# dfdazac/blp

Measured on AMD Instinct MI355X. Metric: scored triples/sec, all-entity eval (raw + filtered ranks, MRR + Hits@k), higher is better.
Workload: dtype f32; 1 GPU; fb15k237-transe; rel_model=transe, entities=14541, dim=128, triples_per_ranking_call=52870, filter_graph_edges=310116, parallelism=single GPU, ranks_in_process_group=1

## Files before the change

blp_amd/csrc/exact_coop.h:

```cpp
#pragma once
#include <hip/hip_runtime.h>
#include <stdint.h>

#include "rank_common.h"
#include "score_core.h"
#include "table_elem.h"

#pragma clang fp contract(off)

namespace blp {

constexpr int kRefStride = 36;

template <class TE>
struct RowOf {
    const TE* p;
    __device__ __forceinline__ float operator[](int k) const { return (float)p[k]; }
};

template <class T>
__device__ __forceinline__ const T* shfl_ptr(const T* p, int src) {
    const unsigned long long v = reinterpret_cast<unsigned long long>(p);
    const unsigned lo = __shfl((unsigned)v, src), hi = __shfl((unsigned)(v >> 32), src);
    return reinterpret_cast<const T*>(((unsigned long long)hi << 32) | lo);
}

template <class T>
__device__ __forceinline__ void gather_chunk(float (&x)[32], const T* const (&g)[8], int s, float* slab, int lane) {
#pragma unroll
    for (int i = 0; i < 8; ++i) {
        const float4 v = load4<T>(g[i] + 32 * s);
        x[4 * i] = v.x; x[4 * i + 1] = v.y; x[4 * i + 2] = v.z; x[4 * i + 3] = v.w;
    }
    float* wr = slab + (lane >> 3) * kRefStride + (lane & 7) * 4;
    wave_lds_sync();
#pragma unroll
    for (int i = 0; i < 8; ++i)
        *reinterpret_cast<float4*>(wr + 8 * i * kRefStride) = make_float4(x[4 * i], x[4 * i + 1], x[4 * i + 2], x[4 * i + 3]);
    wave_lds_sync();
    const float* rd = slab + lane * kRefStride;
#pragma unroll
    for (int j = 0; j < 8; ++j) {
        const float4 w = *reinterpret_cast<const float4*>(rd + 4 * j);
        x[4 * j] = w.x; x[4 * j + 1] = w.y; x[4 * j + 2] = w.z; x[4 * j + 3] = w.w;
    }
}


template <int D, class TE = float>
__device__ __forceinline__ float transe_key_64(const TE* pe, const float* pf, const float* pr, bool head, float* slab, int lane) {
    const int sub_row = lane >> 3, sub_col = (lane & 7) * 4;
    const TE* ge[8];
    const float* gf[8];
    const float* gr[8];
#pragma unroll
    for (int k = 0; k < 8; ++k) {
        ge[k] = shfl_ptr(pe, 8 * k + sub_row) + sub_col;
        gf[k] = shfl_ptr(pf, 8 * k + sub_row) + sub_col;
        gr[k] = shfl_ptr(pr, 8 * k + sub_row) + sub_col;
    }
    float sum = 0.0f;
#pragma unroll
    for (int s = 0; s < D / 32; ++s) {
        float e[32], f[32], r[32];
        gather_chunk(e, ge, s, slab, lane);
        gather_chunk(f, gf, s, slab, lane);
        gather_chunk(r, gr, s, slab, lane);
#pragma unroll
        for (int k = 0; k < 32; ++k) {
            float x = (head ? e[k] : f[k]) + r[k];
            x = x - (head ? f[k] : e[k]);
            sum = sum + fabsf(x);
        }
    }
    return -sum;
}

template <class TE = float>
__device__ __forceinline__ void gather_issue_rt(float (&x)[32], const TE* const (&g)[8], int s, int cols, int lane) {
    const bool mine = (lane & 7) * 4 < cols;
#pragma unroll
    for (int i = 0; i < 8; ++i) {
        float4 v = make_float4(0.f, 0.f, 0.f, 0.f);
        if (mine) v = load4<TE>(g[i] + 32 * s);
        x[4 * i] = v.x; x[4 * i + 1] = v.y; x[4 * i + 2] = v.z; x[4 * i + 3] = v.w;
    }
}
__device__ __forceinline__ void gather_transpose(float (&x)[32], float* slab, int lane) {
    float* wr = slab + (lane >> 3) * kRefStride + (lane & 7) * 4;
    wave_lds_sync();
#pragma unroll
    for (int i = 0; i < 8; ++i)
        *reinterpret_cast<float4*>(wr + 8 * i * kRefStride) = make_float4(x[4 * i], x[4 * i + 1], x[4 * i + 2], x[4 * i + 3]);
    wave_lds_sync();
    const float* rd = slab + lane * kRefStride;
#pragma unroll
    for (int j = 0; j < 8; ++j) {
        const float4 w = *reinterpret_cast<const float4*>(rd + 4 * j);
        x[4 * j] = w.x; x[4 * j + 1] = w.y; x[4 * j + 2] = w.z; x[4 * j + 3] = w.w;
    }
}

__device__ __forceinline__ float transe_key_64_rt(const float* pe, const float* pf, const float* pr, int D, bool head,
                                                  float* slab, int lane) {
    const int sub_row = lane >> 3, sub_col = (lane & 7) * 4;
    const float* ge[8];
    const float* gf[8];
    const float* gr[8];
#pragma unroll
    for (int k = 0; k < 8; ++k) {
        ge[k] = shfl_ptr(pe, 8 * k + sub_row) + sub_col;
        gf[k] = shfl_ptr(pf, 8 * k + sub_row) + sub_col;
        gr[k] = shfl_ptr(pr, 8 * k + sub_row) + sub_col;
    }
    float sum = 0.0f;
    for (int s = 0; s * 32 < D; ++s) {
        const int cols = D - 32 * s < 32 ? D - 32 * s : 32;
        float e[32], f[32], r[32];
        gather_issue_rt(e, ge, s, cols, lane);
        gather_issue_rt(f, gf, s, cols, lane);
        gather_issue_rt(r, gr, s, cols, lane);
        gather_transpose(e, slab, lane);
        gather_transpose(f, slab, lane);
        gather_transpose(r, slab, lane);
#pragma unroll
        for (int k = 0; k < 32; ++k) {
            float x = (head ? e[k] : f[k]) + r[k];
            x = x - (head ? f[k] : e[k]);
            if (k < cols) sum = sum + fabsf(x);
        }
    }
    return -sum;
}

__device__ __forceinline__ void stage_query_rt(const float* __restrict__ f, const float* __restrict__ r, int D, bool head,
                                               float* qa, float* qb, int lane) {
    for (int c = 4 * lane; c < D; c += 256) {
        const float4 fv = *reinterpret_cast<const float4*>(f + c);
        const float4 rv = *reinterpret_cast<const float4*>(r + c);
        if (head) {
            *reinterpret_cast<float4*>(qa + c) = rv;
            *reinterpret_cast<float4*>(qb + c) = fv;
        } else {
            *reinterpret_cast<float4*>(qa + c) = make_float4(fv.x + rv.x, fv.y + rv.y, fv.z + rv.z, fv.w + rv.w);
        }
    }
}

template <class TE = float>
__device__ __forceinline__ float transe_key_64_one_query_rt(const TE* pe, const float* qa, const float* qb, int D, bool head,
                                                            float* slab, int lane) {
    const int sub_row = lane >> 3, sub_col = (lane & 7) * 4;
    const TE* ge[8];
#pragma unroll
    for (int k = 0; k < 8; ++k) ge[k] = shfl_ptr(pe, 8 * k + sub_row) + sub_col;
    float sum = 0.0f;
    const int n_chunks = (D + 31) / 32;
    float ring[4][32];
    auto issue = [&](float (&x)[32], int s) {
        const int rest = D - 32 * s;
        gather_issue_rt(x, ge, s, rest < 32 ? rest : 32, lane);
    };
    auto consume = [&](float (&x)[32], int s) {
        gather_transpose(x, slab, lane);
        const float* a = qa + 32 * s;
        const float* b = qb + 32 * s;
        const int cols = D - 32 * s;
#pragma unroll
        for (int k4 = 0; k4 < 8; ++k4) {
            if (4 * k4 < cols) {
                const float4 av = *reinterpret_cast<const float4*>(a + 4 * k4);
                const float as[4] = {av.x, av.y, av.z, av.w};
                if (head) {
                    const float4 bv = *reinterpret_cast<const float4*>(b + 4 * k4);
                    const float bs[4] = {bv.x, bv.y, bv.z, bv.w};
#pragma unroll
                    for (int i = 0; i < 4; ++i) {
                        float v = x[4 * k4 + i] + as[i];
                        v = v - bs[i];
                        sum = sum + fabsf(v);
                    }
                } else {
#pragma unroll
                    for (int i = 0; i < 4; ++i) sum = sum + fabsf(as[i] - x[4 * k4 + i]);
                }
            }
        }
    };
    if (0 < n_chunks) issue(ring[0], 0);
    if (1 < n_chunks) issue(ring[1], 1);
    if (2 < n_chunks) issue(ring[2], 2);
    for (int s0 = 0; s0 < n_chunks; s0 += 4) {
        static_for<4>([&](auto ii) {
            constexpr int i = decltype(ii)::value;
            const int s = s0 + i;
            if (s < n_chunks) {
                if (s + 3 < n_chunks) issue(ring[(i + 3) % 4], s + 3);
                consume(ring[i], s);
            }
        });
    }
    return -sum;
}

template <int MODEL, int SIDE, int D, class TE>
__device__ __forceinline__ float score_term(const TE* __restrict__ ep, const float* __restrict__ f,
                                            const float* __restrict__ r, int i) {
    constexpr int H = D / 2;
    (void)H;
    const RowOf<TE> e{ep};
    if constexpr (MODEL == DISTMULT) {
        if constexpr (SIDE == TAIL) {
            const float c = f[i] * r[i];
            return c * e[i];
        } else {
            const float x = e[i] * r[i];
            return x * f[i];
        }
    } else if constexpr (MODEL == COMPLEX) {
        if constexpr (SIDE == TAIL) {
            const float c0 = r[i] * f[i], c1 = r[i] * f[H + i], c2 = r[H + i] * f[i], c3 = r[H + i] * f[H + i];
            const float a = c0 * e[i];
            const float b = c1 * e[H + i];
            const float cc = c2 * e[H + i];
            const float d = c3 * e[i];
            float s = a + b;
            s = s + cc;
            return s - d;
        } else {
            float a = r[i] * e[i];          a = a * f[i];
            float b = r[i] * e[H + i];      b = b * f[H + i];
            float cc = r[H + i] * e[i];     cc = cc * f[H + i];
            float d = r[H + i] * e[H + i];  d = d * f[i];
            float s = a + b;
            s = s + cc;
            return s - d;
        }
    } else {
        if constexpr (SIDE == TAIL) {
            const float c0 = f[i] * r[i];
            const float a = c0 * e[H + i];
            float b = e[i] * r[H + i];
            b = b * f[H + i];
            return a + b;
        } else {
            float a = e[i] * r[i];
            a = a * f[H + i];
            const float c2 = f[i] * r[H + i];
            const float b = c2 * e[H + i];
            return a + b;
        }
    }
}

template <int MODEL, int SIDE, int D, class TE = float>
__device__ __forceinline__ float coop_score(const TE* __restrict__ e, const float* __restrict__ f,
                                            const float* __restrict__ r, int sub) {
    constexpr int NT = MODEL == DISTMULT ? D : D / 2;
    float a = score_term<MODEL, SIDE, D>(e, f, r, sub);
#pragma unroll
    for (int k = 1; k < NT / 32; ++k) a = a + score_term<MODEL, SIDE, D>(e, f, r, 32 * k + sub);
    float v = a + __shfl_down(a, 8, 32);
    v = v + __shfl_down(a, 16, 32);
    v = v + __shfl_down(a, 24, 32);
    float s = __shfl(v, 0, 32);
#pragma unroll
    for (int l = 1; l < 8; ++l) s = s + __shfl(v, l, 32);
    return MODEL == SIMPLE ? s / 2.0f : s;
}


template <int MODEL, int D>
__device__ __forceinline__ void true_key_lane(const QRows& q_true, const QRows& q_fixed, const QRows& q_rel,
                                              int64_t q, int64_t q_head, float* __restrict__ key_true,
                                              unsigned long long* __restrict__ acc) {
    acc[q] = 0;
    float e[D];
    load_row<D>(e, q_true.row(q));
    const float* f = q_fixed.row(q);
    const float* r = q_rel.row(q);
    key_true[q] = q < q_head ? Scorer<MODEL, HEAD, D>::template score<false>(e, LazyCoef<MODEL, HEAD, D>{f, r})
                             : Scorer<MODEL, TAIL, D>::template score<false>(e, LazyCoef<MODEL, TAIL, D>{f, r});
}

template <int MODEL, int D>
__device__ __forceinline__ void true_key_lane_side(const QRows& q_true, const QRows& q_fixed, const QRows& q_rel, int64_t q, bool head,
                                                   float* __restrict__ key_true, unsigned long long* __restrict__ acc) {
    acc[q] = 0;
    float e[D];
    load_row<D>(e, q_true.row(q));
    const float* f = q_fixed.row(q);
    const float* r = q_rel.row(q);
    key_true[q] = head ? Scorer<MODEL, HEAD, D>::template score<false>(e, LazyCoef<MODEL, HEAD, D>{f, r})
                       : Scorer<MODEL, TAIL, D>::template score<false>(e, LazyCoef<MODEL, TAIL, D>{f, r});
}

template <int MODEL, int D>
__device__ __forceinline__ void fallback_prep(const FallbackPrep& fp, const QRows& q_fixed, const QRows& q_rel, int64_t q_head,
                                              int64_t q_tail) {
    using SH = Scorer<MODEL, HEAD, D>;
    using ST = Scorer<MODEL, TAIL, D>;
    float* coef_head = fp.coef;
    float* coef_tail = fp.coef + fallback_coef_tail_offset(D, q_head);
    const int64_t stride = (int64_t)gridDim.x * blockDim.x, i0 = blockIdx.x * (int64_t)blockDim.x + threadIdx.x;
    for (int64_t q = i0; q < q_head + q_tail; q += stride) fp.acc[q] = 0;
    const int64_t n_head = q_head * SH::C, total = n_head + q_tail * ST::C;
    for (int64_t i = i0; i < total; i += stride) {
        if (i < n_head) {
            const int64_t q = i / SH::C;
            coef_head[i] = SH::coef(q_fixed.row(q), q_rel.row(q), (int)(i % SH::C));
        } else {
            const int64_t k = i - n_head, q = k / ST::C;
            coef_tail[k] = ST::coef(q_fixed.row(q_head + q), q_rel.row(q_head + q), (int)(k % ST::C));
        }
    }
}

}
```

blp_amd/csrc/rank_sad.hip:

```cpp
#include <hip/hip_runtime.h>
#include <stdint.h>
#include <stdlib.h>

#include "exact_coop.h"
#include "knobs.h"
#include "launch.h"
#include "rank_common.h"
#include "sad_common.h"
#include "score_core.h"

#pragma clang fp contract(off)

namespace blp {


template <int D>
__global__ __launch_bounds__(256) void sad_range_kernel(const float* __restrict__ table, int64_t N, int64_t ld,
                                                        const QRows q_fixed,
                                                        const QRows q_rel, int64_t q_head, int64_t Q,
                                                        SadParams* __restrict__ partial) {
    SadRange range;
    const int64_t stride = (int64_t)gridDim.x * blockDim.x, t0 = (int64_t)blockIdx.x * blockDim.x + threadIdx.x;
    for (int64_t i = t0; i < N * (D / 4); i += stride) {
        const float4 v = *reinterpret_cast<const float4*>(table + (i / (D / 4)) * ld + (i % (D / 4)) * 4);
        range.see(v.x); range.see(v.y); range.see(v.z); range.see(v.w);
    }
    for (int64_t u = t0; u < Q * (D / 4); u += stride) {
        const bool head = u / (D / 4) < q_head;
        const float4 f = *reinterpret_cast<const float4*>(q_fixed.flat(4 * u, D));
        const float4 r = *reinterpret_cast<const float4*>(q_rel.flat(4 * u, D));
        range.see(sad_coef(f.x, r.x, head)); range.see(sad_coef(f.y, r.y, head));
        range.see(sad_coef(f.z, r.z, head)); range.see(sad_coef(f.w, r.w, head));
    }
    sad_range_block_store(range, partial);
}

constexpr int64_t kSFoldFinishBlocks = 1024;
constexpr int64_t kSFoldRangeBlocks = 256;

template <int D>
__device__ __forceinline__ void sad_quantize_table_tile(int64_t tile, const float* __restrict__ table, int64_t N,
                                                        int64_t ld, const SadParams* __restrict__ p,
                                                        uint4* __restrict__ cimg, unsigned* __restrict__ resid) {
    const SadScale sc = sad_scale(p);
    if (!sc.ok) return;
    const int row_in = threadIdx.x >> 2, part = threadIdx.x & 3;
    const int64_t row = tile * 64 + row_in;
    constexpr int F = D / 4;
    unsigned w[F / 2];
    float res = 0.f;
    bool outside = false;
    if (row < N) {
        const float* src = table + row * ld + part * F;
#pragma unroll
        for (int i = 0; i < F / 4; ++i) {
            const float4 v = *reinterpret_cast<const float4*>(src + 4 * i);
            w[2 * i] = sad_quant(v.x, sc, res, outside);
            w[2 * i] |= sad_quant(v.y, sc, res, outside) << 16;
            w[2 * i + 1] = sad_quant(v.z, sc, res, outside);
            w[2 * i + 1] |= sad_quant(v.w, sc, res, outside) << 16;
        }
    } else {
#pragma unroll
        for (int i = 0; i < F / 2; ++i) w[i] = 0;
    }
    res += __shfl_xor(res, 1);
    res += __shfl_xor(res, 2);
    outside |= (bool)__shfl_xor((int)outside, 1);
    outside |= (bool)__shfl_xor((int)outside, 2);
    if (part == 0)
        resid[row] = outside ? kSRowExact : (unsigned)(res * 1.0001f + kSResidSlack * D) + 1u;
    uint4* dst = cimg + (tile * (D / 8) + part * (F / 8)) * 64 + row_in;
#pragma unroll
    for (int i = 0; i < F / 8; ++i) dst[i * 64] = make_uint4(w[4 * i], w[4 * i + 1], w[4 * i + 2], w[4 * i + 3]);
}

template <int D>
__device__ __forceinline__ void sad_quantize_queries_block(int64_t vblock, int64_t vgrid, const QRows& q_fixed,
                                                           const QRows& q_rel, int64_t q_head,
                                                           int64_t Q, const float* __restrict__ key_true,
                                                           const SadParams* __restrict__ p,
                                                           unsigned* __restrict__ qimg,
                                                           int2* __restrict__ thr, unsigned* __restrict__ flags,
                                                           int64_t n_flag_words) {
    const int64_t i = vblock * 256 + threadIdx.x;
    for (int64_t j = i; j < n_flag_words; j += vgrid * 256) flags[j] = 0;
    const SadScale sc = sad_scale(p);
    if (!sc.ok) return;
    __shared__ float part_res[4], part_max[4];
    __shared__ int part_out[4];
    const bool live = i < Q * (D / 2);
    const int64_t q = live ? i / (D / 2) : Q - 1;
    const bool head = q < q_head;
    float res = 0.f, qmax = 0.f;
    bool outside = false;
    if (live) {
        const float2 f = *reinterpret_cast<const float2*>(q_fixed.flat(2 * i, D));
        const float2 r = *reinterpret_cast<const float2*>(q_rel.flat(2 * i, D));
        unsigned w = sad_quant(sad_coef(f.x, r.x, head), sc, res, outside);
        w |= sad_quant(sad_coef(f.y, r.y, head), sc, res, outside) << 16;
        qimg[i] = w;
        qmax = fmaxf(fmaxf(fabsf(f.x), fabsf(f.y)), fmaxf(fabsf(r.x), fabsf(r.y)));
    }
#pragma unroll
    for (int off = 1; off < (D / 2 < 64 ? D / 2 : 64); off <<= 1) {
        res += __shfl_xor(res, off);
        qmax = fmaxf(qmax, __shfl_xor(qmax, off));
        outside |= (bool)__shfl_xor((int)outside, off);
    }
    if constexpr (D / 2 > 64) {
        const int w = threadIdx.x >> 6;
        if ((threadIdx.x & 63) == 0) { part_res[w] = res; part_max[w] = qmax; part_out[w] = outside; }
        __syncthreads();
        res = part_res[w & ~1] + part_res[w | 1];
        qmax = fmaxf(part_max[w & ~1], part_max[w | 1]);
        outside = part_out[w & ~1] || part_out[w | 1];
    }
    if (live && i % (D / 2) == 0) {
        const double u = 5.9604644775390625e-8;
        const double dt = -(double)key_true[q], s = (double)sc.scale;
        const double M = (double)fmaxf(sad_range_maxabs(sc), qmax);
        const double band = (double)res * 1.0001 + 2.0 * kSResidSlack * D + 1.0;
        const double gamma = 1.05 * (D + 2) * u, rho = 6.0 * D * u * M;
        int t_lo = -1, t_hi = (int)kSThrMax;
        if (!outside && M < 3.0e38 && dt >= 0.0 && dt < 1.0e300) {
            const double lo_v = s * (dt - rho) / (1.0 + gamma) - band;
            const double hi_v = s * (dt + rho) / (1.0 - gamma) + band;
            if (lo_v > 2.0) t_lo = lo_v - 1.0 < (double)kSThrMax ? (int)(lo_v - 1.0) : (int)kSThrMax;
            if (hi_v + 2.0 < (double)kSThrMax) t_hi = (int)(hi_v + 2.0);
        }
        thr[q] = make_int2(t_lo, t_hi);
    }
}

template <int D>
__global__ __launch_bounds__(256) void sad_quantize_kernel(const float* __restrict__ table, int64_t N, int64_t ld,
                                                           SadParams* __restrict__ p, const SadParams* __restrict__ partial,
                                                           int n_partial, uint4* __restrict__ cimg,
                                                           unsigned* __restrict__ resid, unsigned table_blocks,
                                                           const QRows q_fixed, const QRows q_rel, int64_t q_head, int64_t Q,
                                                           const float* __restrict__ key_true, unsigned* __restrict__ qimg,
                                                           int2* __restrict__ thr, unsigned* __restrict__ flags,
                                                           int64_t n_flag_words) {
    __shared__ SadParams p_block;
    const SadParams* pp = p;
    if (n_partial > 0) {
        if (threadIdx.x < 64) {
            const SadParams r = sad_range_finish_wave(partial, n_partial, threadIdx.x);
            if (threadIdx.x == 0) {
                p_block = r;
                if (blockIdx.x == 0) *p = r;
            }
        }
        __syncthreads();
        pp = &p_block;
    }
    if (blockIdx.x < table_blocks)
        sad_quantize_table_tile<D>(blockIdx.x, table, N, ld, pp, cimg, resid);
    else
        sad_quantize_queries_block<D>(blockIdx.x - table_blocks, gridDim.x - table_blocks, q_fixed, q_rel, q_head, Q, key_true, pp,
                                      qimg, thr, flags, n_flag_words);
}

template <int D, int TPW>
struct SadTiles {
    unsigned v[TPW][D / 2];
    unsigned bias[TPW];
    unsigned long long exact_rows[TPW];
};

#ifndef BLP_SAD_CHUNK_BLOCK
#define BLP_SAD_CHUNK_BLOCK 4
#endif
constexpr unsigned kSadChunkBlock = BLP_SAD_CHUNK_BLOCK;

#ifdef BLP_TIMING
__device__ unsigned long long g_sad_timing[4];
extern "C" int blp_debug_read_sad_timing(unsigned long long* out) {
    hipError_t err = hipMemcpyFromSymbol(out, HIP_SYMBOL(g_sad_timing), sizeof(g_sad_timing));
    unsigned long long zero[4] = {0, 0, 0, 0};
    if (err == hipSuccess) err = hipMemcpyToSymbol(HIP_SYMBOL(g_sad_timing), zero, sizeof(zero));
    return (int)err;
}
#endif

template <int D, int TPW>
__global__ __launch_bounds__(kSW * 64, (TPW * D / 2 <= 64 ? 5 : TPW * D / 2 <= 128 ? 3 : 2)) void rank_sad_kernel(
    const uint4* __restrict__ cimg, const unsigned* __restrict__ resid, int64_t n_rows, int n_groups, int q_per_group,
    const unsigned* __restrict__ qimg, const int2* __restrict__ thr, int64_t Q, int words_per_query,
    unsigned long long* __restrict__ acc,
    unsigned* __restrict__ flags, uint2* __restrict__ pairs, SadParams* __restrict__ params) {
    if (!sad_scale(params).ok) return;
#ifdef BLP_TIMING
    const unsigned long long clk0 = __builtin_readcyclecounter(), wall0 = __builtin_amdgcn_s_memrealtime();
#endif
    __shared__ int2 thr_s[kSChunk];
    __shared__ unsigned cnt[kSChunk];
    __shared__ uint2 pair_s[kSQuota];
    __shared__ unsigned wave_used[kSW], wave_base[kSW], ec_max_s;
    const int tid = threadIdx.x;
    const int wave = __builtin_amdgcn_readfirstlane(tid >> 6);
    const int lane = tid & 63;
    const unsigned n_blocks = gridDim.x, xcd = blockIdx.x & 7u, per_xcd = n_blocks >> 3, rem_b = n_blocks & 7u;
    const unsigned logical = (xcd < rem_b ? xcd * (per_xcd + 1) : rem_b * (per_xcd + 1) + (xcd - rem_b) * per_xcd) + (blockIdx.x >> 3);
    const unsigned n_chunks_all = n_blocks / (unsigned)n_groups;
    const unsigned per_cb = (unsigned)n_groups * kSadChunkBlock, cb = logical / per_cb, in_cb = logical % per_cb;
    const unsigned chunks_here = n_chunks_all - cb * kSadChunkBlock < kSadChunkBlock ? n_chunks_all - cb * kSadChunkBlock : kSadChunkBlock;
    const int group = (int)(in_cb / chunks_here);
    const int64_t q0 = (int64_t)(cb * kSadChunkBlock + in_cb % chunks_here) * q_per_group;
    const int nq = (int)(Q - q0 < q_per_group ? Q - q0 : q_per_group);

    for (int i = tid; i < kSChunk; i += kSW * 64) cnt[i] = 0;
    if (tid == 0) ec_max_s = 0;
    __syncthreads();

    SadTiles<D, TPW> c;
    const int64_t n_tiles = (n_rows + 63) / 64;
    const int64_t tile0 = ((int64_t)group * kSW + wave) * TPW;
    unsigned ec_max = 0;
    static_for<TPW>([&](auto tt) {
        constexpr int t = decltype(tt)::value;
        int64_t tile = tile0 + t;
        const bool exists = tile * 64 + lane < n_rows;
        tile = tile < n_tiles ? tile : n_tiles - 1;
        const unsigned ec = resid[tile * 64 + lane];
        const bool marked = exists && ec == kSRowExact;
        c.exact_rows[t] = __ballot(marked);
        c.bias[t] = exists ? (marked ? 0u : ec) : kSInvalid;
        ec_max = exists && !marked && ec > ec_max ? ec : ec_max;
        const uint4* src = cimg + tile * (D / 8) * 64 + lane;
        static_for<D / 8>([&](auto jj) {
            constexpr int j = decltype(jj)::value;
            const uint4 x = src[j * 64];
            c.v[t][4 * j] = x.x; c.v[t][4 * j + 1] = x.y; c.v[t][4 * j + 2] = x.z; c.v[t][4 * j + 3] = x.w;
        });
    });
#pragma unroll
    for (int off = 32; off > 0; off >>= 1) {
        const unsigned o = __shfl_xor(ec_max, off);
        ec_max = o > ec_max ? o : ec_max;
    }
    if (lane == 0) atomicMax(&ec_max_s, ec_max);
    __syncthreads();
    for (int i = tid; i < kSChunk; i += kSW * 64) {
        int2 t2 = i < nq ? thr[q0 + i] : make_int2(0, 0);
        const long long hi2 = (long long)t2.y + 2ll * ec_max_s;
        t2.y = hi2 < (long long)kSThrMax ? (int)hi2 : (int)kSThrMax;
        thr_s[i] = t2;
    }
    __syncthreads();

    unsigned my_pairs = 0;
    const float* row = reinterpret_cast<const float*>(qimg + q0 * (D / 2));
    sf16 cur = sload16<0>(row);
    sdrain(cur);
    for (int jb = 0; jb < nq; jb += 64) {
    const int jn = nq - jb < 64 ? nq - jb : 64;
    unsigned cnt_reg = 0;
    unsigned long long bit = 1;
    for (int j = jb; j < jb + jn; ++j, row += D / 2, bit <<= 1) {
        const float* next_row = row + D / 2;
        const int2 th = thr_s[j];
        unsigned sad[TPW];
        static_for<TPW>([&](auto tt) { sad[decltype(tt)::value] = c.bias[decltype(tt)::value]; });
        static_for<D / 32>([&](auto kk) {
            constexpr int k = decltype(kk)::value;
            sf16 nxt;
            if constexpr (k + 1 < D / 32) nxt = sload16<(k + 1) * 64>(row); else nxt = sload16<0>(next_row);
            if constexpr (k == 0) { if ((j & 3) == wave) stouch<D * 2>(row + 3 * (D / 2)); }
            static_for<16>([&](auto ii) {
                constexpr int i = decltype(ii)::value;
                const float qf = cur[i];
                const unsigned qv = __float_as_uint(qf);
                static_for<TPW>([&](auto tt) {
                    constexpr int t = decltype(tt)::value;
                    sad[t] = __builtin_amdgcn_sad_u16(qv, c.v[t][16 * k + i], sad[t]);
                });
            });
            sdrain(nxt);
            cur = nxt;
        });
        unsigned n_above = 0;
        static_for<TPW>([&](auto tt) {
            constexpr int t = decltype(tt)::value;
            const unsigned long long above = __ballot((int)sad[t] < th.x) & ~c.exact_rows[t];
            const unsigned long long und = (__ballot((int)sad[t] <= th.y) | c.exact_rows[t]) & ~above;
            unsigned n_t = __popcll(above);
            if (und) {
                const unsigned n = __popcll(und);
                if (my_pairs + n <= kSQuota / kSW) {
                    if ((und >> lane) & 1ull)
                        pair_s[wave * (kSQuota / kSW) + my_pairs + __popcll(und & ((1ull << lane) - 1ull))] =
                            make_uint2((unsigned)(q0 + j), (unsigned)((tile0 + t) * 64 + lane));
                    my_pairs += n;
                } else {
                    const int64_t tile = tile0 + t;
                    if (lane == 0) atomicOr(flags + (size_t)(q0 + j) * words_per_query + (tile >> 5), 1u << (tile & 31));
                    n_t = 0;
                }
            }
            n_above += n_t;
        });
        {
            unsigned long long saved;
            asm volatile("s_mov_b64 %1, exec\n\ts_mov_b64 exec, %3\n\tv_add_u32 %0, %0, %2\n\ts_mov_b64 exec, %1"
                         : "+v"(cnt_reg), "=&s"(saved) : "s"(n_above), "s"(bit));
        }
    }
    if (cnt_reg) atomicAdd(&cnt[jb + lane], cnt_reg);
    }
    __syncthreads();
    for (int i = tid; i < nq; i += kSW * 64) {
        const unsigned long long v = cnt[i];
        if (v) atomicAdd(acc + q0 + i, v | (v << 32));
    }
    if (lane == 0) wave_used[wave] = my_pairs;
    __syncthreads();
    if (tid == 0) {
        unsigned total = 0;
        for (int w = 0; w < kSW; ++w) { wave_base[w] = total; total += wave_used[w]; }
        const unsigned base = total ? atomicAdd(&params->n_pairs, total) : 0u;
        for (int w = 0; w < kSW; ++w) wave_base[w] += base;
    }
    __syncthreads();
    for (int w = 0; w < kSW; ++w)
        for (unsigned i = tid; i < wave_used[w]; i += kSW * 64) pairs[wave_base[w] + i] = pair_s[w * (kSQuota / kSW) + i];
#ifdef BLP_TIMING
    if (lane == 0) {
        atomicAdd(&g_sad_timing[0], __builtin_readcyclecounter() - clk0);
        atomicAdd(&g_sad_timing[1], __builtin_amdgcn_s_memrealtime() - wall0);
        atomicAdd(&g_sad_timing[2], 1ull);
    }
#endif
}

template <int D>
__global__ __launch_bounds__(64) void sad_refine_pairs_kernel(const float* __restrict__ table, int64_t ld,
                                                              const QRows q_fixed,
                                                              const QRows q_rel,
                                                              const float* __restrict__ key_true, int64_t q_head,
                                                              const uint2* __restrict__ pairs,
                                                              const SadParams* __restrict__ params,
                                                              unsigned long long* __restrict__ acc, const Gate gate) {
    if (gate_heavy(gate)) return;
    __shared__ __attribute__((aligned(16))) float slab[64 * kRefStride];
    const int lane = threadIdx.x;
    const int64_t n = params->n_pairs;
    for (int64_t base = (int64_t)blockIdx.x * 64; base < n; base += (int64_t)gridDim.x * 64) {
        const int64_t i = base + lane;
        const uint2 p = i < n ? pairs[i] : make_uint2(kSNoPair, 0u);
        const bool live = p.x != kSNoPair;
        const int64_t q = live ? p.x : 0;
        const bool head = q < q_head;
        const float key = transe_key_64<D>(table + (live ? (int64_t)p.y : 0) * ld, q_fixed.row(q), q_rel.row(q), head, slab, lane);
        const float kt = key_true[q];
        const unsigned long long gt = live && key > kt, ge_ = live && key >= kt;
        if (gt | ge_) atomicAdd(acc + q, gt | (ge_ << 32));
    }
}

template <int D>
__global__ __launch_bounds__(256) void sad_refine_tiles_kernel(const float* __restrict__ table, int64_t n_rows,
                                                               int64_t ld, const QRows q_fixed,
                                                               const QRows q_rel,
                                                               const float* __restrict__ key_true, int64_t q_head,
                                                               int64_t Q, int words_per_query,
                                                               const unsigned* __restrict__ flags,
                                                               const SadParams* __restrict__ params,
                                                               unsigned long long* __restrict__ acc, const Gate gate,
                                                               const FallbackPrep prep, int64_t q_tail) {
    if (gate_heavy(gate)) {
        fallback_prep<TRANSE, D>(prep, q_fixed, q_rel, q_head, q_tail);
        return;
    }
    __shared__ int list[kSweepQueries], n_list;
    const bool all = !sad_scale(params).ok;
    const int lane = threadIdx.x & 63;
    const int64_t q_base = (int64_t)blockIdx.x * kSweepQueries;
    const int n = flagged_queries(flags, q_base, Q, words_per_query, all, list, &n_list);
    for (int i = threadIdx.x >> 6; i < n; i += 4) {
    const int64_t q = q_base + list[i];
    const unsigned* row = flags + q * words_per_query;
    const float kt = key_true[q];
    const float* f = q_fixed.row(q);
    const float* rl = q_rel.row(q);
    unsigned gt = 0, ge = 0;
    for (int w0 = 0; w0 < words_per_query; w0 += 64) {
        const unsigned mine = w0 + lane < words_per_query ? (all ? 0xFFFFFFFFu : row[w0 + lane]) : 0u;
        unsigned long long nonzero = __ballot(mine != 0);
        while (nonzero) {
            const int src = __builtin_ctzll(nonzero);
            nonzero &= nonzero - 1;
            unsigned bits = __shfl(mine, src);
            const int64_t tile_base = (int64_t)(w0 + src) * 32;
            while (bits) {
                const int b = __builtin_ctz(bits);
                bits &= bits - 1;
                const int64_t r = (tile_base + b) * 64 + lane;
                const bool ok = r < n_rows;
                if (__ballot(ok) == 0) continue;
                float e[D];
                load_row<D>(e, table + (ok ? r : 0) * ld);
                const float key = q < q_head ? Scorer<TRANSE, HEAD, D>::template score<false>(e, LazyCoef<TRANSE, HEAD, D>{f, rl})
                                             : Scorer<TRANSE, TAIL, D>::template score<false>(e, LazyCoef<TRANSE, TAIL, D>{f, rl});
                gt += ok && key > kt;
                ge += ok && key >= kt;
            }
        }
    }
    if (__ballot(gt | ge) == 0) continue;
#pragma unroll
    for (int off = 32; off > 0; off >>= 1) {
        gt += __shfl_down(gt, off);
        ge += __shfl_down(ge, off);
    }
    if (lane == 0) atomicAdd(acc + q, (unsigned long long)gt | ((unsigned long long)ge << 32));
    }
}

static constexpr int sad_tiles_per_wave(int D) { return D <= 64 ? 2 : 1; }

struct SadWorkspace {
    float* key_true;
    unsigned long long* acc;
    SadParams* params; SadParams* partial; int2* thr; unsigned* qimg; uint4* cimg; unsigned* resid; unsigned* flags;
    uint2* pairs;
    float* fallback_coef;
    int64_t pass_groups;
    size_t bytes;
};

static int sad_queries_per_group(int D, int64_t N, int64_t Q) {
    const int64_t tiles_per_group = kSW * sad_tiles_per_wave(D);
    const int64_t n_groups = ((N + 63) / 64 + tiles_per_group - 1) / tiles_per_group;
    const int64_t resident = D >= 256 ? 256 * 3 : 256 * 5;
    const int64_t query_cycles = (int64_t)(D / 2) * sad_tiles_per_wave(D) * 17 / 4, setup_cycles = 12000;
    if (const int forced = (int)knob(KNOB_SAD_QUERIES_PER_GROUP))
        if (forced >= 16 && forced <= kSChunk && (forced & (forced - 1)) == 0) return forced;
    int best = kSChunk;
    int64_t best_cost = INT64_MAX;
    for (int per_group = kSChunk; per_group >= 16; per_group >>= 1) {
        const int64_t grid = n_groups * ((Q + per_group - 1) / per_group);
        const int64_t cost = ((grid + resident - 1) / resident) * (setup_cycles + per_group * query_cycles);
        if (cost < best_cost) { best_cost = cost; best = per_group; }
    }
    return best;
}

static int64_t sad_groups_per_pass(int D, int64_t N, int64_t Q) {
    const int64_t tiles_per_group = kSW * sad_tiles_per_wave(D);
    const int64_t n_groups = ((N + 63) / 64 + tiles_per_group - 1) / tiles_per_group;
    const int64_t per_group = sad_queries_per_group(D, N, Q);
    const int64_t n_chunks = (Q + per_group - 1) / per_group;
    const int64_t cap = (int64_t)256 << 20;
    int64_t by_pairs = cap / (kSQuota * 8) / (n_chunks > 0 ? n_chunks : 1);
    int64_t by_flags = cap / 4 / (Q > 0 ? Q : 1) * 32 / tiles_per_group;
    int64_t g = n_groups;
    if (g > by_pairs) g = by_pairs;
    if (g > by_flags) g = by_flags;
    if (const int64_t forced = knob(KNOB_SAD_PASS_GROUPS))
        if (forced > 0 && forced < g) g = forced;
    return g < 1 ? 1 : g;
}

static SadWorkspace carve_sad(void* base, int D, int64_t N, int64_t q_head, int64_t q_tail) {
    SadWorkspace w;
    const int64_t Q = q_head + q_tail;
    char* p = static_cast<char*>(base);
    size_t off = 0;
    w.key_true = reinterpret_cast<float*>(p + off);  off = align_up(off + (size_t)Q * 4, 256);
    w.acc = reinterpret_cast<unsigned long long*>(p + off);   off = align_up(off + (size_t)Q * 8, 256);
    w.params = reinterpret_cast<SadParams*>(p + off); off = align_up(off + sizeof(SadParams), 256);
    w.partial = reinterpret_cast<SadParams*>(p + off); off = align_up(off + sizeof(SadParams) * kSRangeBlocks, 256);
    w.thr = reinterpret_cast<int2*>(p + off);         off = align_up(off + (size_t)Q * 8, 256);
    w.qimg = reinterpret_cast<unsigned*>(p + off);    off = align_up(off + (size_t)(Q + 4) * (D / 2) * 4 + 64, 256);
    w.cimg = reinterpret_cast<uint4*>(p + off);       off = align_up(off + (size_t)((N + 63) / 64) * 64 * (D / 2) * 4, 256);
    w.resid = reinterpret_cast<unsigned*>(p + off);   off = align_up(off + (size_t)((N + 63) / 64) * 64 * 4, 256);
    w.pass_groups = sad_groups_per_pass(D, N, Q);
    const int64_t tiles_per_group = kSW * sad_tiles_per_wave(D);
    const int64_t words = (w.pass_groups * tiles_per_group + 31) / 32;
    w.flags = reinterpret_cast<unsigned*>(p + off); off = align_up(off + (size_t)Q * words * 4, 256);
    w.pairs = reinterpret_cast<uint2*>(p + off);
    const int64_t per_group = sad_queries_per_group(D, N, Q);
    off = align_up(off + (size_t)w.pass_groups * ((Q + per_group - 1) / per_group) * kSQuota * 8, 256);
    w.fallback_coef = nullptr;
    const int64_t n_groups_all = ((N + 63) / 64 + tiles_per_group - 1) / tiles_per_group;
    if (w.pass_groups >= n_groups_all && Q * N >= kFallbackMinPairs && Q <= 0x7fffffff / 2) {
        w.fallback_coef = reinterpret_cast<float*>(p + off);
        off = align_up(off + exact_fallback_coef_floats(D, q_head, q_tail) * 4, 256);
    }
    w.bytes = off;
    return w;
}

bool rank_sad_applicable(int model, int D, int64_t N, int64_t q_head, int64_t q_tail) {
    if (knob(KNOB_RANK_KERNEL) == 1) return false;
    const int64_t Q = q_head + q_tail;
    int64_t min_queries = kSadMinQueries;
    bool forced = false;
    if (const int64_t v = knob(KNOB_SAD_MIN_QUERIES)) { min_queries = v > 0 ? v : 1; forced = true; }
    if (model != TRANSE || !(D == 64 || D == 128 || D == 256) || Q < min_queries) return false;
    return forced || Q * N >= kSadMinPairs;
}

hipError_t sad_prepass_stats(int D, int64_t N, int64_t q_head, int64_t q_tail, const void* workspace, PrepassStats* out,
                             hipStream_t stream) {
    const SadWorkspace w = carve_sad(const_cast<void*>(workspace), D, N, q_head, q_tail);
    out->path = 1;
    const int64_t tiles_per_group = kSW * sad_tiles_per_wave(D);
    const int64_t words = (w.pass_groups * tiles_per_group + 31) / 32;
    unsigned long long host[3] = {0, 0, 0};
    const hipError_t err = launch_count_bits(w.flags, (q_head + q_tail) * words, w.pairs, &w.params->n_pairs, false, host, stream);
    out->flagged_rows = (long long)host[0] * 64;
    out->listed = (long long)host[2];
    return err;
}

size_t rank_sad_workspace_bytes(int model, int D, int64_t N, int64_t q_head, int64_t q_tail) {
    if (!rank_sad_applicable(model, D, N, q_head, q_tail)) return 0;
    return carve_sad(nullptr, D, N, q_head, q_tail).bytes;
}

template <int D>
static hipError_t rank_sad_impl(const float* table, int64_t N, int64_t ld, const QRows q_fixed, const QRows q_rel,
                                const QRows q_true, int64_t q_head, int64_t q_tail,
                                const FilterSpec& filter, int32_t* counts, void* workspace,
                                int n_cu, hipStream_t stream, hipEvent_t ev_start, hipEvent_t ev_stop) {
    constexpr int TPW = sad_tiles_per_wave(D);
    const int64_t Q = q_head + q_tail;
    SadWorkspace w = carve_sad(workspace, D, N, q_head, q_tail);
    hipError_t err = launch_true_keys(TRANSE, D, q_fixed, q_rel, q_head, q_tail, q_true, w.key_true, w.acc,
                                      stream);
    if (err != hipSuccess) return err;
    if (ev_start) (void)hipEventRecord(ev_start, stream);
    const int64_t n_tiles = (N + 63) / 64;
    const int64_t query_blocks = (Q * (D / 2) + 255) / 256;
    if (n_tiles + query_blocks > 0x7fffffff) return hipErrorInvalidValue;
    const bool fold_finish = n_tiles + query_blocks <= kSFoldFinishBlocks;
    int64_t range_blocks;
    {
        const int64_t items = N * (D / 4) > Q * D ? N * (D / 4) : Q * D, cap = fold_finish ? kSFoldRangeBlocks : kSRangeBlocks;
        range_blocks = (items + 255) / 256;
        range_blocks = range_blocks < cap ? (range_blocks > 0 ? range_blocks : 1) : cap;
        sad_range_kernel<D><<<dim3((unsigned)range_blocks), 256, 0, stream>>>(table, N, ld, q_fixed, q_rel, q_head, Q, w.partial);
        if (!fold_finish) sad_range_finish_kernel<<<1, 64, 0, stream>>>(w.partial, (int)range_blocks, w.params);
    }
    const int64_t first_rows = N < w.pass_groups * kSW * TPW * 64 ? N : w.pass_groups * kSW * TPW * 64;
    const int64_t first_groups = ((first_rows + 63) / 64 + kSW * TPW - 1) / (kSW * TPW);
    const int64_t first_words = (first_groups * kSW * TPW + 31) / 32;
    sad_quantize_kernel<D><<<dim3((unsigned)(n_tiles + query_blocks)), 256, 0, stream>>>(
        table, N, ld, w.params, w.partial, fold_finish ? (int)range_blocks : 0, w.cimg, w.resid, (unsigned)n_tiles, q_fixed, q_rel,
        q_head, Q, w.key_true, w.qimg, w.thr, w.flags, first_words * Q);

    const int64_t tiles_per_group = kSW * TPW;
    const int per_group = sad_queries_per_group(D, N, Q);
    const int64_t n_chunks = (Q + per_group - 1) / per_group;
    const int64_t pass_rows = w.pass_groups * tiles_per_group * 64;
    for (int64_t slab0 = 0; slab0 < N; slab0 += pass_rows) {
        const int64_t n_rows = N - slab0 < pass_rows ? N - slab0 : pass_rows;
        const int64_t slab_tiles = (n_rows + 63) / 64;
        const int64_t n_groups = (slab_tiles + tiles_per_group - 1) / tiles_per_group;
        const int words = (int)((n_groups * tiles_per_group + 31) / 32);
        const int64_t n_blocks = n_groups * n_chunks;
        if (slab0 > 0) {
            err = hipMemsetAsync(w.flags, 0, (size_t)Q * words * 4, stream);
            if (err != hipSuccess) return err;
            err = hipMemsetAsync(&w.params->n_pairs, 0, 4, stream);
            if (err != hipSuccess) return err;
        }
        const float* slab = table + slab0 * ld;
        rank_sad_kernel<D, TPW><<<dim3((unsigned)n_blocks), kSW * 64, 0, stream>>>(
            w.cimg + (slab0 / 64) * (D / 8) * 64, w.resid + slab0, n_rows, (int)n_groups, per_group, w.qimg, w.thr, Q, words, w.acc,
            w.flags, w.pairs, w.params);
        const int64_t pair_blocks = (n_blocks * kSQuota + 63) / 64;
        const Gate gate{w.fallback_coef ? &w.params->n_pairs : nullptr, (unsigned)((n_blocks * kSQuota / 10 * 9) < 0xffffffffll ? n_blocks * kSQuota / 10 * 9 : 0xffffffffll)};
        sad_refine_pairs_kernel<D><<<dim3((unsigned)(pair_blocks < (int64_t)n_cu * 40 ? pair_blocks : (int64_t)n_cu * 40)), 64, 0, stream>>>(
            slab, ld, q_fixed, q_rel, w.key_true, q_head, w.pairs, w.params, w.acc, gate);
        sad_refine_tiles_kernel<D><<<dim3((unsigned)((Q + kSweepQueries - 1) / kSweepQueries)), 256, 0, stream>>>(
            slab, n_rows, ld, q_fixed, q_rel, w.key_true, q_head, Q, words, w.flags, w.params, w.acc, gate,
            FallbackPrep{w.fallback_coef, w.acc}, q_tail);
        if (gate.counter) {
            err = launch_exact_fallback(TRANSE, D, table, N, ld, q_fixed, q_rel, q_head, q_tail, w.fallback_coef, w.key_true, w.acc, gate,
                                        n_cu, stream);
            if (err != hipSuccess) return err;
        }
    }
    if (ev_stop) (void)hipEventRecord(ev_stop, stream);
    err = launch_filter_finalize(TRANSE, D, table, N, ld, q_fixed, q_rel, w.key_true, q_head, q_tail, filter,
                                 w.acc, counts, stream);
    return err != hipSuccess ? err : hipGetLastError();
}

hipError_t launch_rank_all_sad(int D, const float* table, int64_t N, int64_t ld, const QRows q_fixed,
                               const QRows q_rel, const QRows q_true, int64_t q_head,
                               int64_t q_tail, const FilterSpec& filter, int32_t* counts,
                               void* workspace, int n_cu, hipStream_t stream, hipEvent_t ev_start,
                               hipEvent_t ev_stop) {
#define BLP_SAD_CASE(DD)                                                                                          \
    if (D == DD)                                                                                                  \
        return rank_sad_impl<DD>(table, N, ld, q_fixed, q_rel, q_true, q_head, q_tail, filter,          \
                                 counts, workspace, n_cu, stream, ev_start, ev_stop);
    BLP_SAD_CASE(64) BLP_SAD_CASE(128) BLP_SAD_CASE(256)
#undef BLP_SAD_CASE
    return hipErrorInvalidValue;
}

}
```

blp_amd/csrc/sad_common.h:

```cpp
#pragma once
#include <hip/hip_runtime.h>
#include <stdint.h>

#pragma clang fp contract(off)

namespace blp {

constexpr int kSW = 4;
constexpr int kSChunk = 256;
constexpr int kSadMinQueries = 64;
constexpr long long kSadMinPairs = 4000000;
constexpr int kSQuota = 1024;
constexpr unsigned kSInvalid = 0x40001000u;
constexpr unsigned kSThrMax = 0x3fffffffu;
constexpr unsigned kSNoPair = 0xFFFFFFFFu;

constexpr unsigned kSRowExact = 0xFFFFFFFFu;

struct SadParams {
    int lo_ord, hi_ord;
    unsigned nonfinite;
    unsigned n_pairs;
    double sum, sumsq;
    unsigned long long count;
};
constexpr int kSRangeBlocks = 1024;
constexpr float kSClampSigmas = 16.0f;

__device__ __forceinline__ int f2ord(float f) { const int b = __float_as_int(f); return b >= 0 ? b : b ^ 0x7fffffff; }
__device__ __forceinline__ float ord2f(int o) { return __int_as_float(o >= 0 ? o : o ^ 0x7fffffff); }

struct SadScale { float lo, hi, scale; bool ok; };

__device__ __forceinline__ SadScale sad_scale(const SadParams* __restrict__ p) {
    SadScale s;
    const int lo_ord = p->lo_ord, hi_ord = p->hi_ord;
    s.lo = ord2f(lo_ord);
    s.hi = ord2f(hi_ord);
    const float range = s.hi - s.lo;
    s.scale = 65535.0f / range;
    s.ok = lo_ord <= hi_ord && range > 0.f && range < 3.0e38f && s.scale > 0.f && s.scale < 3.0e38f;
    return s;
}
__device__ __forceinline__ float sad_range_maxabs(const SadScale& s) { return fmaxf(fabsf(s.lo), fabsf(s.hi)); }

__device__ __forceinline__ unsigned sad_quant(float x, const SadScale& s, float& resid, bool& outside) {
    outside |= !(x >= s.lo && x <= s.hi);
    const float v = fminf(fmaxf((x - s.lo) * s.scale, 0.f), 65535.f);
    const float r = rintf(v);
    resid += fabsf(v - r);
    return (unsigned)r;
}
constexpr float kSResidSlack = 0.0079f;

__device__ __forceinline__ float sad_coef(float fixed, float rel, bool head) { return head ? fixed - rel : fixed + rel; }

struct SadRange {
    int lo = 0x7fffffff, hi = (int)0x80000000;
    unsigned bad = 0;
    double sum = 0.0, sumsq = 0.0;
    unsigned long long count = 0;
    __device__ __forceinline__ void see(float x) {
        if (!(fabsf(x) < 3.0e38f)) { ++bad; return; }
        const int o = f2ord(x);
        lo = o < lo ? o : lo;
        hi = o > hi ? o : hi;
        sum += (double)x;
        sumsq += (double)x * (double)x;
        ++count;
    }
    __device__ __forceinline__ void merge(int lo2, int hi2, unsigned bad2, double sum2, double sumsq2, unsigned long long count2) {
        lo = lo2 < lo ? lo2 : lo;
        hi = hi2 > hi ? hi2 : hi;
        bad += bad2; sum += sum2; sumsq += sumsq2; count += count2;
    }
    __device__ __forceinline__ void wave_reduce() {
#pragma unroll
        for (int off = 32; off > 0; off >>= 1)
            merge(__shfl_xor(lo, off), __shfl_xor(hi, off), __shfl_xor(bad, off), __shfl_xor(sum, off), __shfl_xor(sumsq, off),
                  __shfl_xor(count, off));
    }
    __device__ __forceinline__ SadParams record() const {
        SadParams p = {};
        p.lo_ord = lo; p.hi_ord = hi; p.nonfinite = bad; p.sum = sum; p.sumsq = sumsq; p.count = count;
        return p;
    }
};

__device__ __forceinline__ void sad_range_block_store(SadRange r, SadParams* __restrict__ partial) {
    __shared__ SadParams part[4];
    r.wave_reduce();
    if ((threadIdx.x & 63) == 0) part[threadIdx.x >> 6] = r.record();
    __syncthreads();
    if (threadIdx.x == 0) {
        SadRange t;
        for (int w = 0; w < 4; ++w) t.merge(part[w].lo_ord, part[w].hi_ord, part[w].nonfinite, part[w].sum, part[w].sumsq, part[w].count);
        partial[blockIdx.x] = t.record();
    }
}

__device__ __forceinline__ SadParams sad_range_finish_wave(const SadParams* __restrict__ partial, int n, int lane) {
    SadRange r;
    for (int i = lane; i < n; i += 64) {
        const SadParams p = partial[i];
        r.merge(p.lo_ord, p.hi_ord, p.nonfinite, p.sum, p.sumsq, p.count);
    }
    r.wave_reduce();
    SadParams p = r.record();
    p.n_pairs = 0;
    if (r.count > 0 && r.lo <= r.hi) {
        const double mean = r.sum / (double)r.count;
        const double var = r.sumsq / (double)r.count - mean * mean;
        const double sd = var > 0.0 ? sqrt(var) : 0.0;
        const float lo_c = (float)(mean - kSClampSigmas * sd), hi_c = (float)(mean + kSClampSigmas * sd);
        if (lo_c > ord2f(r.lo)) p.lo_ord = f2ord(lo_c);
        if (hi_c < ord2f(r.hi)) p.hi_ord = f2ord(hi_c);
    }
    return p;
}

static __global__ __launch_bounds__(64) void sad_range_finish_kernel(const SadParams* __restrict__ partial, int n,
                                                              SadParams* __restrict__ out) {
    const SadParams p = sad_range_finish_wave(partial, n, threadIdx.x);
    if (threadIdx.x == 0) *out = p;
}

}
```

Before: 489.6 billion scored triples/s.

## Refine small per-block candidate lists inline in the SAD rank kernel

When a block's flagged candidate pairs number at most a cap, wave 0 of that block now computes the exact TransE key for each pair itself and atomically updates the rank counters. Only blocks with larger lists still write their pairs to global memory for the separate refine kernel. This avoids global pair traffic and refine work for most blocks. It adds a serial per-lane 128-dim exact score on one wave while the other waves sit idle, a new n_listed counter for the gate and stats, and an extra host sync to read that counter in the stats path.

```diff
diff --git a/blp_amd/csrc/exact_coop.h b/blp_amd/csrc/exact_coop.h
--- a/blp_amd/csrc/exact_coop.h
+++ b/blp_amd/csrc/exact_coop.h
@@ -71,6 +71,35 @@
             float x = (head ? e[k] : f[k]) + r[k];
             x = x - (head ? f[k] : e[k]);
             sum = sum + fabsf(x);
+        }
+    }
+    return -sum;
+}
+
+template <int D>
+__device__ __forceinline__ float transe_key_lane(const float* pe, const float* pf, const float* pr, bool head) {
+    const float* pa = head ? pe : pf;
+    const float* pb = head ? pf : pe;
+    float sum = 0.0f;
+#pragma unroll 1
+    for (int c = 0; c < D; c += 16) {
+        float4 a[4], r[4], b[4];
+#pragma unroll
+        for (int i = 0; i < 4; ++i) a[i] = *reinterpret_cast<const float4*>(pa + c + 4 * i);
+#pragma unroll
+        for (int i = 0; i < 4; ++i) r[i] = *reinterpret_cast<const float4*>(pr + c + 4 * i);
+#pragma unroll
+        for (int i = 0; i < 4; ++i) b[i] = *reinterpret_cast<const float4*>(pb + c + 4 * i);
+#pragma unroll
+        for (int i = 0; i < 4; ++i) {
+            const float av[4] = {a[i].x, a[i].y, a[i].z, a[i].w}, rv[4] = {r[i].x, r[i].y, r[i].z, r[i].w},
+                        bv[4] = {b[i].x, b[i].y, b[i].z, b[i].w};
+#pragma unroll
+            for (int k = 0; k < 4; ++k) {
+                float x = av[k] + rv[k];
+                x = x - bv[k];
+                sum = sum + fabsf(x);
+            }
         }
     }
     return -sum;
diff --git a/blp_amd/csrc/rank_sad.hip b/blp_amd/csrc/rank_sad.hip
--- a/blp_amd/csrc/rank_sad.hip
+++ b/blp_amd/csrc/rank_sad.hip
@@ -1,4 +1,5 @@
 #include <hip/hip_runtime.h>
+#include <stddef.h>
 #include <stdint.h>
 #include <stdlib.h>
 
@@ -174,6 +175,12 @@
 #endif
 constexpr unsigned kSadChunkBlock = BLP_SAD_CHUNK_BLOCK;
 
+#ifndef BLP_SAD_INLINE_CAP
+#define BLP_SAD_INLINE_CAP 256
+#endif
+constexpr unsigned kSInlineCap = BLP_SAD_INLINE_CAP;
+static_assert(kSInlineCap <= kSQuota, "the pooled list is the four slices of pair_s");
+
 #ifdef BLP_TIMING
 __device__ unsigned long long g_sad_timing[4];
 extern "C" int blp_debug_read_sad_timing(unsigned long long* out) {
@@ -189,7 +196,9 @@
     const uint4* __restrict__ cimg, const unsigned* __restrict__ resid, int64_t n_rows, int n_groups, int q_per_group,
     const unsigned* __restrict__ qimg, const int2* __restrict__ thr, int64_t Q, int words_per_query,
     unsigned long long* __restrict__ acc,
-    unsigned* __restrict__ flags, uint2* __restrict__ pairs, SadParams* __restrict__ params) {
+    unsigned* __restrict__ flags, uint2* __restrict__ pairs, SadParams* __restrict__ params,
+    const float* __restrict__ table, int64_t ld, const QRows q_fixed, const QRows q_rel, int64_t q_head,
+    const float* __restrict__ key_true) {
     if (!sad_scale(params).ok) return;
 #ifdef BLP_TIMING
     const unsigned long long clk0 = __builtin_readcyclecounter(), wall0 = __builtin_amdgcn_s_memrealtime();
@@ -316,15 +325,36 @@
     }
     if (lane == 0) wave_used[wave] = my_pairs;
     __syncthreads();
-    if (tid == 0) {
-        unsigned total = 0;
-        for (int w = 0; w < kSW; ++w) { wave_base[w] = total; total += wave_used[w]; }
-        const unsigned base = total ? atomicAdd(&params->n_pairs, total) : 0u;
-        for (int w = 0; w < kSW; ++w) wave_base[w] += base;
-    }
-    __syncthreads();
-    for (int w = 0; w < kSW; ++w)
-        for (unsigned i = tid; i < wave_used[w]; i += kSW * 64) pairs[wave_base[w] + i] = pair_s[w * (kSQuota / kSW) + i];
+    unsigned start[kSW + 1];
+    start[0] = 0;
+#pragma unroll
+    for (int w = 0; w < kSW; ++w) start[w + 1] = start[w] + __builtin_amdgcn_readfirstlane(wave_used[w]);
+    const unsigned total = start[kSW];
+    if (tid == 0 && total) atomicAdd(&params->n_listed, total);
+    if (total <= kSInlineCap) {
+        if (wave == 0) {
+            for (unsigned base = 0; base < total; base += 64) {
+                const bool live = base + lane < total;
+                const unsigned t = live ? base + lane : base;
+                const unsigned w = (unsigned)(t >= start[1]) + (unsigned)(t >= start[2]) + (unsigned)(t >= start[3]);
+                const unsigned first = w == 0 ? start[0] : w == 1 ? start[1] : w == 2 ? start[2] : start[3];
+                const uint2 p = pair_s[w * (kSQuota / kSW) + (t - first)];
+                const int64_t q = p.x;
+                const float key = transe_key_lane<D>(table + (int64_t)p.y * ld, q_fixed.row(q), q_rel.row(q), q < q_head);
+                const float kt = key_true[q];
+                const unsigned long long gt = live && key > kt, ge_ = live && key >= kt;
+                if (gt | ge_) atomicAdd(acc + q, gt | (ge_ << 32));
+            }
+        }
+    } else {
+        if (tid == 0) {
+            const unsigned base = atomicAdd(&params->n_pairs, total);
+            for (int w = 0; w < kSW; ++w) wave_base[w] = base + start[w];
+        }
+        __syncthreads();
+        for (int w = 0; w < kSW; ++w)
+            for (unsigned i = tid; i < wave_used[w]; i += kSW * 64) pairs[wave_base[w] + i] = pair_s[w * (kSQuota / kSW) + i];
+    }
 #ifdef BLP_TIMING
     if (lane == 0) {
         atomicAdd(&g_sad_timing[0], __builtin_readcyclecounter() - clk0);
@@ -512,8 +542,12 @@
     unsigned long long host[3] = {0, 0, 0};
     const hipError_t err = launch_count_bits(w.flags, (q_head + q_tail) * words, w.pairs, &w.params->n_pairs, false, host, stream);
     out->flagged_rows = (long long)host[0] * 64;
-    out->listed = (long long)host[2];
-    return err;
+    if (err != hipSuccess) return err;
+    unsigned n_listed = 0;
+    hipError_t err2 = hipMemcpyAsync(&n_listed, &w.params->n_listed, 4, hipMemcpyDeviceToHost, stream);
+    if (err2 == hipSuccess) err2 = hipStreamSynchronize(stream);
+    out->listed = (long long)n_listed;
+    return err2;
 }
 
 size_t rank_sad_workspace_bytes(int model, int D, int64_t N, int64_t q_head, int64_t q_tail) {
@@ -565,15 +599,16 @@
         if (slab0 > 0) {
             err = hipMemsetAsync(w.flags, 0, (size_t)Q * words * 4, stream);
             if (err != hipSuccess) return err;
-            err = hipMemsetAsync(&w.params->n_pairs, 0, 4, stream);
+            static_assert(offsetof(SadParams, n_listed) == offsetof(SadParams, n_pairs) + 4, "one memset clears both counters");
+            err = hipMemsetAsync(&w.params->n_pairs, 0, 8, stream);
             if (err != hipSuccess) return err;
         }
         const float* slab = table + slab0 * ld;
         rank_sad_kernel<D, TPW><<<dim3((unsigned)n_blocks), kSW * 64, 0, stream>>>(
             w.cimg + (slab0 / 64) * (D / 8) * 64, w.resid + slab0, n_rows, (int)n_groups, per_group, w.qimg, w.thr, Q, words, w.acc,
-            w.flags, w.pairs, w.params);
+            w.flags, w.pairs, w.params, slab, ld, q_fixed, q_rel, q_head, w.key_true);
         const int64_t pair_blocks = (n_blocks * kSQuota + 63) / 64;
-        const Gate gate{w.fallback_coef ? &w.params->n_pairs : nullptr, (unsigned)((n_blocks * kSQuota / 10 * 9) < 0xffffffffll ? n_blocks * kSQuota / 10 * 9 : 0xffffffffll)};
+        const Gate gate{w.fallback_coef ? &w.params->n_listed : nullptr, (unsigned)((n_blocks * kSQuota / 10 * 9) < 0xffffffffll ? n_blocks * kSQuota / 10 * 9 : 0xffffffffll)};
         sad_refine_pairs_kernel<D><<<dim3((unsigned)(pair_blocks < (int64_t)n_cu * 40 ? pair_blocks : (int64_t)n_cu * 40)), 64, 0, stream>>>(
             slab, ld, q_fixed, q_rel, w.key_true, q_head, w.pairs, w.params, w.acc, gate);
         sad_refine_tiles_kernel<D><<<dim3((unsigned)((Q + kSweepQueries - 1) / kSweepQueries)), 256, 0, stream>>>(
diff --git a/blp_amd/csrc/sad_common.h b/blp_amd/csrc/sad_common.h
--- a/blp_amd/csrc/sad_common.h
+++ b/blp_amd/csrc/sad_common.h
@@ -19,10 +19,11 @@
 
 struct SadParams {
     int lo_ord, hi_ord;
-    unsigned nonfinite;
     unsigned n_pairs;
+    unsigned n_listed;
     double sum, sumsq;
     unsigned long long count;
+    unsigned nonfinite;
 };
 constexpr int kSRangeBlocks = 1024;
 constexpr float kSClampSigmas = 16.0f;
@@ -107,7 +108,7 @@
     }
     r.wave_reduce();
     SadParams p = r.record();
-    p.n_pairs = 0;
+    p.n_pairs = p.n_listed = 0;
     if (r.count > 0 && r.lo <= r.hi) {
         const double mean = r.sum / (double)r.count;
         const double var = r.sumsq / (double)r.count - mean * mean;
```

Measured after the change: 506.2 billion scored triples/s, median of 6. 1.03x the previous value.
